# microsoft/Nova

Measured on NVIDIA H100. Metric: MSM throughput (2^20 BN254 scalar*G1/s), higher is better.
Workload: dtype u32 limbs (256-bit prime-field / curve integers)

## Files before the change

### nova_b200/csrc/capi.cu

```cuda
#include <cuda_runtime.h>

#include <algorithm>
#include <atomic>
#include <cstdarg>
#include <cstdio>
#include <cstring>
#include <cstdlib>
#include <map>
#include <memory>
#include <mutex>
#include <vector>

#include "../../include/nova_b200.h"
#include "msm_kernels.cuh"
#include "field_kernels.cuh"
#include "ops.cuh"
#include "poly_kernels.cuh"
#include "transcript.cuh"
#include "transcript_batched.cuh"
#include "sumcheck_tail.cuh"

using namespace nova;

namespace {
// ... 225 lines not shown
size_t acc_lmin() {
  static const size_t lmin = [] {
    const char* e = getenv("NOVA_B200_ACC_LMIN");
    int v = e ? atoi(e) : L_FLOOR_DEFAULT;
    return (size_t)(v < 8 ? 8 : (v > L_MIN ? L_MIN : v));
  }();
  return lmin;
}
int segment_len(size_t entries) {
  size_t L = (entries + acc_threads() - 1) / acc_threads();
  return (int)(L < acc_lmin() ? acc_lmin() : L);
}
size_t max_segments(size_t entries) {
  size_t by_floor = (entries + acc_lmin() - 1) / acc_lmin();
  size_t cap = acc_threads() + 256;
  return by_floor < cap ? by_floor : cap;
}

int ws_acquire(workspace& w, cudaStream_t s) {
  if (w.busy && w.last_stream != s) CU(cudaStreamWaitEvent(s, w.busy, 0));
  return B200_OK;
}
int ws_release(workspace& w, cudaStream_t s) {
  if (!w.busy) CU(cudaEventCreateWithFlags(&w.busy, cudaEventDisableTiming));
  CU(cudaEventRecord(w.busy, s));
  w.last_stream = s;
  return B200_OK;
}

int ensure_workspace(ck_ctx& ck, workspace& w, size_t n, size_t out_slots) {
  if (out_slots > w.out_slots) {
    if (w.d_out) cudaFree(w.d_out);
    if (w.h_out) cudaFreeHost(w.h_out);
    w.d_out = w.h_out = nullptr;
    CU(cudaMalloc(&w.d_out, out_slots * 96));
    CU(cudaMallocHost(&w.h_out, out_slots * 96));
    w.out_slots = out_slots;
  }
  if (n <= w.cap_n) return B200_OK;
  if (n * (size_t)ck.W > 0x7FFFFFFFu)
    return fail(B200_E_RANGE, "%zu scalars x %d windows exceed 2^31 bucket entries", n, ck.W);
  CU(cudaDeviceSynchronize());
  void** szbufs[] = {&w.scalars, (void**)&w.digits, (void**)&w.entries, (void**)&w.entries_tmp, (void**)&w.look,
                     &w.parts, (void**)&w.pkeys, (void**)&w.heavy, &w.hparts};
  for (void** p : szbufs)
    if (*p) {
      cudaFree(*p);
      *p = nullptr;
    }
  size_t K = (size_t)ck.G * ck.B;
  size_t entries = n * (size_t)ck.W;
  size_t nseg = max_segments(entries);
  w.heavy_cap = (uint32_t)(nseg / HEAVY_PARTS + 2);
  CU(cudaMalloc((void**)&w.heavy, ((size_t)w.heavy_cap + 1) * 4));
  CU(cudaMalloc(&w.hparts, (size_t)w.heavy_cap * HEAVY_SPLIT * XYZZ_BYTES));
  CU(cudaMalloc(&w.scalars, n * 32));
  CU(cudaMalloc((void**)&w.digits, entries * sizeof(int32_t)));
  CU(cudaMalloc((void**)&w.entries, entries * sizeof(uint64_t)));
  CU(cudaMalloc((void**)&w.entries_tmp, entries * sizeof(uint64_t)));
  const size_t look_bytes = (entries + SORT_TILE - 1) / SORT_TILE * SORT_BINS * sizeof(unsigned long long);
  CU(cudaMalloc((void**)&w.look, look_bytes));
  CU(cudaMemset(w.look, 0, look_bytes));
  w.sort_epoch = 0;
  CU(cudaMalloc(&w.parts, 2 * nseg * XYZZ_BYTES));
  CU(cudaMalloc((void**)&w.pkeys, 2 * nseg * sizeof(uint32_t)));
  if (!w.sortctl) {
    CU(cudaMalloc((void**)&w.sortctl, SORT_CTL_WORDS * 4));
    CU(cudaMalloc((void**)&w.start, (K + 1) * 4));
    CU(cudaMalloc(&w.buckets, K * XYZZ_BYTES));
    CU(cudaMalloc(&w.rparts, ((size_t)ck.G * (ck.B / ck.m + 4096)) * XYZZ_BYTES));
    CU(cudaMalloc(&w.sumscratch, (size_t)SUM_THREADS * XYZZ_BYTES));
  }
  w.cap_n = n;
  return B200_OK;
}

int ensure_workspace(ck_ctx& ck, size_t n, size_t out_slots) {
  return ensure_workspace(ck, ck.ws, n, out_slots);
}

msm_plan make_plan(ck_ctx& ck, workspace& ws, size_t base_offset, size_t n) {
  msm_plan p;
  p.n = n;
  p.n_ck = ck.stride;
  p.base_offset = base_offset;
  p.blind_i = SIZE_MAX;
  p.h_index = ck.n;
  p.c = ck.c;
  p.W = ck.W;
  p.G = ck.G;
  p.B = ck.B;
  p.L = segment_len(n * (size_t)ck.W);
  p.m = ck.m;
  p.heavy = ws.heavy;
  p.heavy_min = HEAVY_PARTS * (uint32_t)p.L;
  p.heavy_cap = ws.heavy_cap;
  p.hparts = ws.hparts;
  p.digits = ws.digits;
  p.sortctl = ws.sortctl;
  p.sp = make_sort_plan((uint64_t)ck.G * ck.B);
  p.sort_tag = 0;
  p.look = ws.look;
  p.start = ws.start;
  p.entries = ws.entries;
  p.entries_tmp = ws.entries_tmp;
  p.buckets = ws.buckets;
  p.parts = ws.parts;
  p.pkeys = ws.pkeys;
  p.rparts = ws.rparts;
  return p;
}

int enqueue_msm(ck_ctx& ck, workspace& ws, size_t base_offset, const void* d_scalars, size_t n,
                void* d_out, cudaStream_t s, int small_elem_bytes = 0, bool blinded = false,
                bool digits_done = false, const msm_peer* peer = nullptr, bool profile_ok = true) {
  const field_ops* sops = ops_for_field(CURVES[ck.curve].scalar_fid);
  const field_ops* bops = ops_for_field(CURVES[ck.curve].base_fid);
  {
    int arc = ws_acquire(ws, s);
    if (arc) return arc;
  }
  if (n == 0) {
    if (peer && peer->world > 1) {
      msm_plan p0 = make_plan(ck, ws, base_offset, 0);
      p0.peer = *peer;
      bops->exchange_identity(s, p0, d_out);
      count_launch(1);
      CU(cudaGetLastError());
      return B200_OK;
    }
    CU(cudaMemsetAsync(d_out, 0, 96, s));
    return B200_OK;
  }
  msm_plan p = make_plan(ck, ws, base_offset, n);
  if (peer) p.peer = *peer;
  if (blinded) p.blind_i = n - 1;
  if (!digits_done) CU(cudaMemsetAsync(p.sortctl, 0, SORT_CTL_WORDS * 4, s));
  else CU(cudaMemsetAsync(p.sortctl + SORT_PASSES_MAX * SORT_BINS, 0, SORT_PASSES_MAX * 4, s));
  CU(cudaMemsetAsync(p.heavy, 0, 4, s));
  if (ws.sort_epoch > 0x7FFFFFFFu - SORT_PASSES_MAX) {
    CU(cudaMemsetAsync(ws.look, 0, (ws.cap_n * (size_t)ck.W + SORT_TILE - 1) / SORT_TILE * SORT_BINS * 8, s));
    ws.sort_epoch = 0;
  }
  p.sort_tag = ws.sort_epoch + 1;
  ws.sort_epoch += (uint32_t)p.sp.passes;
  std::lock_guard<std::mutex> plk(g_prof.mu);
  const bool prof = g_prof.enabled && profile_ok;
  const int pset = g_prof.next;
  if (prof) {
    if (!g_prof.have_events) {
      for (auto& set : g_prof.ev)
        for (auto& e : set) CU(cudaEventCreate(&e));
      g_prof.have_events = true;
    }
    prof_fold_set_locked(pset);
    g_prof.next = (pset + 1) % profile_state::PROF_RING;
  }
#define STAGE_MARK(i) \
  if (prof) CU(cudaEventRecord(g_prof.ev[pset][i], s))
  STAGE_MARK(ST_DIGITS);
  if (digits_done)
    ;
  else if (small_elem_bytes)
    msm_digits_small(s, d_scalars, small_elem_bytes, p);
  else
    sops->digits(s, d_scalars, p);
  STAGE_MARK(ST_SORT);
  const int sort_launches = msm_sort(s, p);
  STAGE_MARK(ST_ACCUMULATE);
  bops->accumulate(s, ck.tables, p);
  STAGE_MARK(ST_FIXUP);
  bops->fixup(s, p);
  STAGE_MARK(ST_REDUCE);
  bops->reduce(s, p, d_out);
  STAGE_MARK(ST_COUNT);
#undef STAGE_MARK
  if (prof) g_prof.pending[pset] = true;
  for (int i = 0; i < ST_COUNT; i++) g_prof.launches += STAGE_KERNELS[i];
  g_prof.launches += sort_launches - STAGE_KERNELS[ST_SORT];
  g_prof.launches += (ck.c - 1 + 3) / 4 - 1;
  CU(cudaGetLastError());
  return ws_release(ws, s);
}

int enqueue_msm(ck_ctx& ck, size_t base_offset, const void* d_scalars, size_t n, void* d_out,
                cudaStream_t s, int small_elem_bytes = 0, bool blinded = false) {
  return enqueue_msm(ck, ck.ws, base_offset, d_scalars, n, d_out, s, small_elem_bytes, blinded);
}

constexpr size_t SMALL_KEY_MAX = (size_t)1 << 21;
constexpr int SMALL_KEY_WINDOW = 17;

int choose_window(size_t n) {
  int lg = 0;
  while (((size_t)1 << lg) < n) lg++;
  int c = lg;
  if (c < 8) c = 8;
  if (c > 16) c = 16;
  if (lg >= 22) c = 20;
  else if (lg >= 19) c = 17;
  return c;
}

constexpr int CURVE_B_SMALL[4] = {3, -17, 5, 5};

int register_key(int curve_id, const void* bases, bool bases_on_device, size_t n, const void* h,
                 int window_bits, bool expand, std::shared_ptr<ck_ctx>& out, size_t* first_bad = nullptr,
                 cudaStream_t st = nullptr, size_t src_pitch_points = 0, size_t src_block_points = 0) {
  if (!st) st = g_dev.stream;
  if (curve_id < 0 || curve_id > 3) return fail(B200_E_ARG, "unknown curve id %d", curve_id);
  if (bases == nullptr || n == 0) return fail(B200_E_ARG, "empty commitment key");
  if (window_bits != 0 && (window_bits < 2 || window_bits > 24))
    return fail(B200_E_ARG, "window_bits %d out of range [2,24]", window_bits);
  auto ck = std::make_shared<ck_ctx>();
  ck->curve = curve_id;
  ck->n = n;
  ck->has_h = h != nullptr;
  ck->stride = n + (h ? 1 : 0);
  ck->c = window_bits ? window_bits : choose_window(n);
  int bits = FIELD_BITS[CURVES[curve_id].scalar_fid];
  ck->W = (bits + ck->c - 1) / ck->c;
  ck->F = expand ? ck->W : 1;
  ck->G = expand ? 1 : ck->W;
  ck->B = 1u << (ck->c - 1);
  ck->m = ck->B >= 4 ? 4 : 1;
  if ((size_t)ck->F * ck->stride >= ((size_t)1 << 31))
    return fail(B200_E_RANGE, "key too large for 31-bit table indices (%zu x %d)", n, ck->F);
  CU(cudaMalloc(&ck->tables, (size_t)ck->F * ck->stride * 64));
  const cudaMemcpyKind kind = bases_on_device ? cudaMemcpyDeviceToDevice : cudaMemcpyHostToDevice;
  if (src_block_points == 0) {
    CU(cudaMemcpyAsync(ck->tables, bases, n * 64, kind, st));
  } else {
    const size_t full = n / src_block_points, rest = n % src_block_points;
// ... 1400 lines not shown
```

### nova_b200/csrc/curve.cuh

```cuda
#pragma once
#include "field.cuh"

namespace nova {

struct xyzz_t {
  fe_t x, y, zz, zzz;
};

struct affine_t {
  fe_t x, y;
};

template <class F>
NOVA_HD xyzz_t xyzz_identity() {
  xyzz_t r;
  r.x = fe_one<F>();
  r.y = fe_one<F>();
  r.zz = fe_zero<F>();
  r.zzz = fe_zero<F>();
  return r;
}

NOVA_HD bool xyzz_is_identity(const xyzz_t& p) { return fe_is_zero(p.zz); }
NOVA_HD bool affine_is_identity(const affine_t& p) { return fe_is_zero(p.x) && fe_is_zero(p.y); }
// ... 90 lines not shown
    if (fe_eq(s1, s2))
      xyzz_dbl<F>(acc);
    else
      acc = xyzz_identity<F>();
    return;
  }
  fe_t p = fe_sub<F>(u2, u1);
  fe_t r = fe_sub<F>(s2, s1);
  fe_t pp = fe_sqr<F>(p);
  fe_t ppp = fe_mul<F>(p, pp);
  fe_t q = fe_mul<F>(u1, pp);
  fe_t x3 = fe_sub<F>(fe_sub<F>(fe_sqr<F>(r), ppp), fe_dbl<F>(q));
  fe_t y3 = fe_sub<F>(fe_mul<F>(r, fe_sub<F>(q, x3)), fe_mul<F>(s1, ppp));
  acc.x = x3;
  acc.y = y3;
  acc.zz = fe_mul<F>(fe_mul<F>(acc.zz, o.zz), pp);
  acc.zzz = fe_mul<F>(fe_mul<F>(acc.zzz, o.zzz), ppp);
}

template <class F>
NOVA_HD void xyzz_neg(xyzz_t& p) {
  p.y = fe_neg<F>(p.y);
}

template <class F>
NOVA_HD void xyzz_to_jacobian(const xyzz_t& p, fe_t& X, fe_t& Y, fe_t& Z) {
  if (xyzz_is_identity(p)) {
    X = fe_zero<F>();
    Y = fe_one<F>();
    Z = fe_zero<F>();
    return;
  }
  fe_t zzz2 = fe_sqr<F>(p.zzz);
  fe_t zz_zzz2 = fe_mul<F>(p.zz, zzz2);
  X = fe_mul<F>(p.x, zz_zzz2);
  fe_t zz2 = fe_sqr<F>(p.zz);
  Y = fe_mul<F>(p.y, fe_mul<F>(zz2, zz_zzz2));
  Z = fe_mul<F>(p.zz, p.zzz);
}

template <class F>
NOVA_HD xyzz_t xyzz_mul_small(const xyzz_t& p, uint32_t k) {
  xyzz_t acc = xyzz_identity<F>();
  if (k == 0 || xyzz_is_identity(p)) return acc;
  int top = 31;
  while (!((k >> top) & 1)) top--;
  for (int i = top; i >= 0; i--) {
    xyzz_dbl<F>(acc);
    if ((k >> i) & 1) xyzz_add<F>(acc, p);
  }
  return acc;
}

#if defined(__CUDACC__)
NOVA_D affine_t affine_load(const void* base, size_t idx) {
  affine_t a;
  a.x = fe_load(base, 2 * idx);
  a.y = fe_load(base, 2 * idx + 1);
  return a;
}
NOVA_D xyzz_t xyzz_load(const void* base, size_t idx) {
  xyzz_t p;
  p.x = fe_load_rw(base, 4 * idx);
  p.y = fe_load_rw(base, 4 * idx + 1);
  p.zz = fe_load_rw(base, 4 * idx + 2);
  p.zzz = fe_load_rw(base, 4 * idx + 3);
  return p;
}
NOVA_D void xyzz_store(void* base, size_t idx, const xyzz_t& p) {
  fe_store(base, 4 * idx, p.x);
  fe_store(base, 4 * idx + 1, p.y);
  fe_store(base, 4 * idx + 2, p.zz);
  fe_store(base, 4 * idx + 3, p.zzz);
}
#endif

}
```

### nova_b200/csrc/msm_kernels.cuh

```cuda
#pragma once
#include <cuda_runtime.h>
#include "curve29.cuh"
#include "coop.cuh"
#include "msm_sort.cuh"

namespace nova {

constexpr uint32_t KEY_INVALID = 0xffffffffu;

constexpr int MSM_PEER_MAX = 8;
constexpr size_t MSM_PEER_FLAGS_OFF = (size_t)2 * MSM_PEER_MAX * 128;
constexpr size_t MSM_PEER_ERR_OFF = MSM_PEER_FLAGS_OFF + (size_t)MSM_PEER_MAX * 8;
constexpr size_t MSM_PEER_BUF_BYTES = MSM_PEER_ERR_OFF + 8;
struct msm_peer {
  int world = 1, rank = 0;
  unsigned long long epoch = 0;
  void* buf[MSM_PEER_MAX] = {};
};

struct msm_plan {
  size_t n;
  size_t n_ck;
  size_t base_offset;
  size_t blind_i;
  size_t h_index;
  int c;
  int W;
  int G;
  uint32_t B;
  int L;
  int m;
  int32_t* digits;
  uint32_t* sortctl;
  sort_plan sp;
  uint32_t sort_tag;
  unsigned long long* look;
  uint32_t* start;
  uint64_t* entries;
  uint64_t* entries_tmp;
  void* buckets;
  void* parts;
  uint32_t* pkeys;
  void* rparts;
  uint32_t* heavy;
  uint32_t heavy_min;
  uint32_t heavy_cap;
  void* hparts;
  msm_peer peer;
};

template <class S>
__global__ void __launch_bounds__(256) k_digits(const void* __restrict__ scalars, size_t i0, size_t i1,
                                                size_t n, int c, int W, int G, uint32_t B,
                                                int32_t* __restrict__ digits,
                                                uint32_t* __restrict__ hist, const sort_plan sp) {
  __shared__ uint32_t s_hist[SORT_PASSES_MAX * SORT_BINS];
  sort_hist_clear(s_hist);
  for (size_t blk = i0 + (size_t)blockIdx.x * blockDim.x; blk < i1; blk += (size_t)gridDim.x * blockDim.x) {
    size_t i = blk + threadIdx.x;
    const bool live = i < i1;
    fe_t s = live ? fe_from_mont<S>(fe_load(scalars, i)) : fe_zero<S>();
    uint32_t p[8], t[8];
    load_p<S>(p);
    bool neg = false;
    if (!fe_is_zero(s)) {
      sub8(t, p, s.l);
      uint32_t d[8];
      uint32_t lt = sub8(d, t, s.l);
      if (lt) {
        neg = true;
#pragma unroll
        for (int k = 0; k < 8; k++) s.l[k] = t[k];
      }
    }
    const uint32_t half = 1u << (c - 1);
    const uint32_t mask = (1u << c) - 1;
    uint32_t carry = 0;
    for (int w = 0; w < W; w++) {
      int bit = w * c;
      int limb = bit >> 5, sh = bit & 31;
      uint32_t v = 0;
      if (limb < 8) {
        uint64_t two = s.l[limb];
        if (limb + 1 < 8) two |= (uint64_t)s.l[limb + 1] << 32;
        v = (uint32_t)(two >> sh) & mask;
      }
      v += carry;
      int32_t dgt;
      if (v > half) {
        dgt = (int32_t)v - (int32_t)(1u << c);
        carry = 1;
      } else {
        dgt = (int32_t)v;
        carry = 0;
      }
      if (neg) dgt = -dgt;
      if (live) digits[(size_t)w * n + i] = dgt;
      uint32_t key = NO_KEY;
      if (dgt != 0) {
        uint32_t mag = dgt < 0 ? (uint32_t)(-dgt) : (uint32_t)dgt;
        key = (uint32_t)(w % G) * B + (mag - 1);
      }
// ... 643 lines not shown
  for (int s = 32; s > 0; s >>= 1) {
    if (quad < s && s < nsplit) {
      xyzz_t o = sm[quad + s];
      coop_add<F>(acc, o, cm);
    }
    __syncthreads();
    if (quad < s && cm.lane() == 0) sm[quad] = acc;
    __syncthreads();
  }
  if (threadIdx.x == 0) xyzz_store(merged, ((size_t)g * lv.nd + d) * 16 + v, acc);
}

template <class F>
NOVA_D xyzz_t peer_exchange_sum(const xyzz_t& mine, const msm_peer& peer, xyzz_t* sm ,
                                const quad_comm_dev& cm) {
  const int tid = threadIdx.x, quad = tid >> 2;
  const int set = (int)(peer.epoch & 1ull);
  if (tid == 0) sm[0] = mine;
  __syncthreads();
  if (tid < peer.world) {
    char* dst = (char*)peer.buf[tid];
    xyzz_store(dst, (size_t)set * MSM_PEER_MAX + peer.rank, sm[0]);
    __threadfence_system();
    volatile unsigned long long* flag = (volatile unsigned long long*)(dst + MSM_PEER_FLAGS_OFF) + peer.rank;
    *flag = peer.epoch;
    char* loc = (char*)peer.buf[peer.rank];
    const unsigned long long* lflag = (const unsigned long long*)(loc + MSM_PEER_FLAGS_OFF) + tid;
    unsigned long long seen = 0;
    long long t0 = clock64();
    for (;;) {
      asm volatile("ld.acquire.sys.global.u64 %0, [%1];" : "=l"(seen) : "l"(lflag) : "memory");
      if (seen >= peer.epoch) break;
      if (clock64() - t0 > (1ll << 32)) {
        *(volatile unsigned long long*)(loc + MSM_PEER_ERR_OFF) = peer.epoch;
        break;
      }
    }
  }
  __syncthreads();
  xyzz_t acc = xyzz_identity<F>();
  if (quad < peer.world) acc = xyzz_load((const char*)peer.buf[peer.rank], (size_t)set * MSM_PEER_MAX + quad);
  for (int s = MSM_PEER_MAX / 2; s > 0; s >>= 1) {
    if (quad < 2 * s && cm.lane() == 0) sm[quad] = acc;
    __syncthreads();
    if (quad < s && quad + s < peer.world) {
      xyzz_t o = sm[quad + s];
      coop_add<F>(acc, o, cm);
    }
    __syncthreads();
  }
  return acc;
}

template <class F>
__global__ void __launch_bounds__(384) k_red_final_q(const void* __restrict__ merged, int G, int bits, int c,
                                                     void* __restrict__ out_jac, const msm_peer peer) {
  __shared__ xyzz_t sm[96];
  quad_comm_dev cm;
  const int nd = (bits + 3) / 4;
  const int quad = threadIdx.x >> 2;
  const int d = quad >> 4, v = quad & 15;
  xyzz_t total = xyzz_identity<F>();
  for (int g = G - 1; g >= 0; g--) {
    xyzz_t acc = xyzz_identity<F>();
    if (d < nd) acc = xyzz_load(merged, ((size_t)g * nd + d) * 16 + v);
    if (cm.lane() == 0) sm[quad] = acc;
    __syncthreads();
    for (int dd = 1; dd < 16; dd <<= 1) {
      bool have = v + dd < 16;
      xyzz_t o = xyzz_identity<F>();
      if (have) o = sm[quad + dd];
      __syncthreads();
      if (have) coop_add<F>(acc, o, cm);
      if (cm.lane() == 0) sm[quad] = acc;
      __syncthreads();
    }
    xyzz_t t0 = acc;
    if (v == 0) acc = xyzz_identity<F>();
    if (cm.lane() == 0) sm[quad] = acc;
    __syncthreads();
    for (int s = 8; s > 0; s >>= 1) {
      bool have = v < s;
      xyzz_t o = xyzz_identity<F>();
      if (have) o = sm[quad + s];
      __syncthreads();
      if (have) coop_add<F>(acc, o, cm);
      if (cm.lane() == 0) sm[quad] = acc;
      __syncthreads();
    }
    if (v == 0 && d < nd) {
      for (int i = 0; i < 4 * d; i++) coop_dbl<F>(acc, cm);
      if (d == 0) coop_add<F>(acc, t0, cm);
      if (cm.lane() == 0) sm[quad] = acc;
    }
    __syncthreads();
    if (quad == 0) {
      if (g != G - 1)
        for (int i = 0; i < c; i++) coop_dbl<F>(total, cm);
      for (int dd = 0; dd < nd; dd++) {
        xyzz_t o = sm[dd * 16];
        coop_add<F>(total, o, cm);
      }
    }
    __syncthreads();
  }
  if (peer.world > 1) total = peer_exchange_sum<F>(total, peer, sm, cm);
  if (threadIdx.x == 0) {
    fe_t X, Y, Z;
    xyzz_to_jacobian<F>(total, X, Y, Z);
    fe_store(out_jac, 0, X);
    fe_store(out_jac, 1, Y);
    fe_store(out_jac, 2, Z);
  }
}
#endif

template <class F>
__global__ void k_jacobian_sum(const void* __restrict__ pts, int k, void* __restrict__ out_jac) {
  using PA = msm_arith<F>;
  if (blockIdx.x != 0 || threadIdx.x != 0) return;
  typename PA::pt acc = PA::identity();
  for (int i = 0; i < k; i++) {
    fe_t X = fe_load(pts, 3 * (size_t)i), Y = fe_load(pts, 3 * (size_t)i + 1),
         Z = fe_load(pts, 3 * (size_t)i + 2);
    typename PA::pt p = PA::from_jacobian_std(X, Y, Z);
    PA::add(acc, p);
  }
  fe_t X, Y, Z;
  PA::to_jacobian_std(acc, X, Y, Z);
  fe_store(out_jac, 0, X);
  fe_store(out_jac, 1, Y);
  fe_store(out_jac, 2, Z);
}

#if !defined(NOVA_MSM_ARITH29)
template <class F>
__global__ void __launch_bounds__(32) k_jacobian_sum_q(const void* __restrict__ pts, int k, void* __restrict__ out_jac) {
  __shared__ xyzz_t sm[8];
  quad_comm_dev cm;
  const int quad = threadIdx.x >> 2;
  xyzz_t acc = xyzz_identity<F>();
  for (int i = quad; i < k; i += 8) {
    fe_t X = fe_load(pts, 3 * (size_t)i), Y = fe_load(pts, 3 * (size_t)i + 1), Z = fe_load(pts, 3 * (size_t)i + 2);
    xyzz_t p = xyzz_identity<F>();
    if (!fe_is_zero(Z)) {
      p.x = X;
      p.y = Y;
      p.zz = fe_sqr<F>(Z);
      p.zzz = fe_mul<F>(p.zz, Z);
    }
    coop_add<F>(acc, p, cm);
  }
  for (int s = 4; s > 0; s >>= 1) {
    if (quad < 2 * s && cm.lane() == 0) sm[quad] = acc;
    __syncwarp();
    if (quad < s) {
      xyzz_t o = sm[quad + s];
      coop_add<F>(acc, o, cm);
// ... 127 lines not shown
```

### nova_b200/csrc/ops.cuh

```cuda
#pragma once
#include <cstdlib>
#include <cuda_runtime.h>
#include <cstddef>
#include <cstdint>

namespace nova {

struct msm_plan;
struct multi_args;
struct poly_multi_args;
struct scb_tail_args;
struct spark_mats;
struct r1cs_mats;

struct field_ops {
  int field_id;
  void (*digits)(cudaStream_t, const void* scalars, const msm_plan&);
  void (*expand_key)(cudaStream_t, void* tables, size_t n_ck, int ntables, int shift);
  void (*accumulate)(cudaStream_t, const void* tables, const msm_plan&);
  void (*fixup)(cudaStream_t, const msm_plan&);
  void (*reduce)(cudaStream_t, const msm_plan&, void* out_jac);
  void (*sum_points)(cudaStream_t, const void* tables, const uint32_t* idx_or_null, size_t n,
                     void* scratch_xyzz, void* out_jac);
  void (*jacobian_sum)(cudaStream_t, const void* pts, int k, void* out_jac);
  void (*index_bases)(cudaStream_t, void* bases, size_t n, const void* gen_affine, uint64_t k0);
  void (*cross_term)(cudaStream_t, const void* az, const void* bz, const void* cz, const void* e1,
                     const void* e2_or_null, const void* u, size_t n, void* t);
  void (*axpy)(cudaStream_t, const void* a, const void* b, const void* r, size_t n, void* out);
  void (*vec_add)(cudaStream_t, const void* a, const void* b, size_t n, void* out);
  void (*bind_top)(cudaStream_t, void* z, size_t n, const void* r);
  void (*bind_top_multi)(cudaStream_t, void* const* zs, int k, size_t n, const void* r);
  void (*vec_mul)(cudaStream_t, const void* a, const void* b, size_t n, void* out);
  void (*logup_hash)(cudaStream_t, const void* val, const void* addr_or_null, const void* gamma,
                     const void* r, size_t n, void* out);
  void (*fold_halves)(cudaStream_t, const void* v, size_t half, const void* x_lo, const void* x_hi, void* out);
  void (*ipa_scalars)(cudaStream_t, const void* a, const void* w, size_t n, size_t nk, void* sL, void* sR);
  void (*ipa_weights)(cudaStream_t, void* w, size_t n, size_t nk, const void* r, const void* r_inv);
  void (*fill_one)(cudaStream_t, void* w, size_t n);
  void (*sc_reduce)(cudaStream_t, int form, const void* A, const void* B, const void* C, size_t count,
                    size_t half, const void* eq_left, const void* eq_right, int shift, size_t id_mul,
                    size_t id_add, void* scratch, void* out);
  void (*eq_small)(cudaStream_t, const void* r, int ell, void* out);
  void (*eq_outer)(cudaStream_t, const void* left, const void* right, int right_bits, size_t n,
                   void* out);
  void (*batch_invert)(cudaStream_t, const void* in, size_t n, void* out, int* zero_flag);
  void (*rlc)(cudaStream_t, const void* const* polys, const size_t* lens, int k, const void* coeffs,
              size_t n, void* out);
  void (*kzg_fold)(cudaStream_t, const void* p, const void* x, size_t half, void* out);
  void (*poly_eval)(cudaStream_t, const void* f, size_t n, const void* us, int nu, void* scratch,
                    void* evals);
  void (*poly_div)(cudaStream_t, const void* f, size_t n, size_t cols, const void* u, void* scratch, void* out,
                   void* rem_or_null);
  void (*spmv_classify)(cudaStream_t, const void* vals, size_t nnz, int8_t* codes);
  void (*spmv)(cudaStream_t, const uint32_t* indptr, const uint32_t* cols, const int8_t* codes,
               const void* vals, size_t rows, const void* z1, const void* z2_or_null, void* o1,
               void* o2_or_null);
  void (*spmv_t)(cudaStream_t, const uint32_t* tptr, const uint32_t* trow, const uint32_t* tperm,
                 const int8_t* codes, const void* vals, size_t cols, size_t out_len, const void* rx,
                 void* out);
  void (*sc_round)(cudaStream_t, int kind, void* state, const void* res, const void* tau,
                   const void* tau_inv, const void* pending, uint32_t pending_len, int absorb_label,
                   int squeeze_label, void* out_poly, void* out_r);
  void (*fe_inv_each)(cudaStream_t, const void* in, size_t n, void* out);
  void (*digits_range)(cudaStream_t, const void* scalars, size_t i0, size_t i1, const msm_plan&);
  void (*sc_round_batched)(cudaStream_t, const void* desc, void* state, const void* sums, const void* pending,
                           uint32_t pending_len, int absorb_label, int squeeze_label, void* out_poly, void* out_r);
  void (*on_curve)(cudaStream_t, const void* pts, size_t n, int b_small, uint32_t* first_bad);
  void (*powers_canonical)(cudaStream_t, const void* u_mont, size_t n, void* out);
  void (*scalar_bases)(cudaStream_t, void* bases, size_t n, const void* gen_affine, const void* scalars_canonical);
  void (*poseidon_ro)(cudaStream_t, int t, int r_f, int r_p, const void* rc, const void* mds, const void* elems, uint32_t n,
                      const void* tag_canonical, int num_bits, int start_with_one, void* out);
  void (*to_mont)(cudaStream_t, const void* in_canonical, size_t n, void* out);
  void (*exchange_identity)(cudaStream_t, const msm_plan&, void* out_jac);
  void (*sc_round_batched_fused)(cudaStream_t, const void* desc, void* state, const void* partials, int nblocks,
// ... 78 lines not shown
```

### nova_b200/csrc/ops_impl.cuh

```cuda
#pragma once
#include "ops.cuh"
#include "msm_kernels.cuh"
#include "field_kernels.cuh"
#include "poly_kernels.cuh"
#include "transcript.cuh"
#include "transcript_batched.cuh"
#include "poseidon.cuh"
#include "sumcheck_tail.cuh"

namespace nova {

inline int stream_grid(size_t n, int block, int waves = 8) {
  size_t need = (n + block - 1) / block;
  size_t cap = (size_t)NUM_SMS * waves;
  size_t g = need < cap ? need : cap;
  return (int)(g == 0 ? 1 : g);
}

template <class F>
__global__ void __launch_bounds__(128) k_sum_points1(const void* __restrict__ tables,
                                                     const uint32_t* __restrict__ idx, size_t n,
                                                     void* __restrict__ partial) {
  size_t tid = (size_t)blockIdx.x * blockDim.x + threadIdx.x;
  size_t nthreads = (size_t)gridDim.x * blockDim.x;
// ... 22 lines not shown
    int block = 128;
    int grid = (int)((n_ck + block - 1) / block);
    k_expand_key<F><<<grid, block, 0, s>>>(tables, n_ck, ntables, shift);
  }
  static void accumulate(cudaStream_t s, const void* tables, const msm_plan& p) {
    uint32_t K = (uint32_t)p.G * p.B;
    size_t max_entries = p.n * (size_t)p.W;
    size_t nseg = (max_entries + p.L - 1) / p.L;
    int block = 128;
    int grid = (int)((nseg + block - 1) / block);
#if !defined(NOVA_MSM_ARITH29)
    static const bool use_tma = [] {
      const char* e = getenv("NOVA_B200_ACC_TMA");
      return e != nullptr && e[0] == '1';
    }();
    if (use_tma) {
      k_accumulate_tma<F><<<grid, block, 0, s>>>(p.entries, p.start, K, tables, p.L, p.buckets, p.parts, p.pkeys);
      return;
    }
#endif
    k_accumulate<F><<<grid, block, 0, s>>>(p.entries, p.start, K, tables, p.L, p.buckets, p.parts,
                                           p.pkeys);
  }
  static void fixup(cudaStream_t s, const msm_plan& p) {
    uint32_t K = (uint32_t)p.G * p.B;
    size_t entries = p.n * (size_t)p.W;
    size_t ppk = entries / ((size_t)K * p.L) + 1;
    int G = 1;
    while (G < 32 && (size_t)G * 8 < ppk) G <<= 1;
    if (ppk <= 16) G = 1;
    size_t threads = (size_t)K * G;
#if !defined(NOVA_MSM_ARITH29)
    if (G == 1) {
      threads = (size_t)K * 4;
      k_fixup_q<F><<<(unsigned)((threads + 127) / 128), 128, 0, s>>>(p.start, K, p.L, p.heavy_min, p.parts,
                                                                     p.pkeys, p.buckets);
    } else
#endif
      k_fixup<F><<<(unsigned)((threads + 127) / 128), 128, 0, s>>>(p.start, K, p.L, p.heavy_min, G, p.parts,
                                                                   p.pkeys, p.buckets);
    k_fixup_heavy1<F><<<NUM_SMS * 4, 256, 0, s>>>(p.start, p.L, p.heavy, p.parts, p.pkeys, p.hparts);
    k_fixup_heavy2<F><<<NUM_SMS, 32, 0, s>>>(p.heavy, p.hparts, p.buckets);
  }
  static void index_bases(cudaStream_t s, void* bases, size_t n, const void* gen, uint64_t k0) {
    k_index_bases<F><<<(unsigned)((n + 127) / 128), 128, 0, s>>>(bases, n, gen, k0);
  }
  static void jacobian_sum(cudaStream_t s, const void* pts, int k, void* out_jac) {
#if !defined(NOVA_MSM_ARITH29)
    k_jacobian_sum_q<F><<<1, 32, 0, s>>>(pts, k, out_jac);
#else
    k_jacobian_sum<F><<<1, 32, 0, s>>>(pts, k, out_jac);
#endif
  }
  static void reduce(cudaStream_t s, const msm_plan& p, void* out_jac) {
    int bits = p.c - 1;
#if !defined(NOVA_MSM_ARITH29)
    static const int flat_mode = [] {
      const char* e = getenv("NOVA_B200_RED_FLAT");
      return e == nullptr ? -1 : (e[0] == '1' ? 1 : 0);
    }();
    static const int hier_bits = [] {
      const char* e = getenv("NOVA_B200_RED_HIER_BITS");
      return e ? atoi(e) : 18;
    }();
    const bool flat = flat_mode == 1 || (flat_mode == -1 && bits < hier_bits);
    if (bits >= 1 && bits <= 24 && !flat) {
      red_levels lv{};
      lv.nd = (bits + 3) / 4;
      size_t off = 0;
      uint32_t N = p.B;
      const void* X = p.buckets;
      for (int l = 0; l < lv.nd - 1; l++) {
        const uint32_t groups = N >> 4;
        int nsplit = (int)((groups + 511) / 512);
        if (nsplit < 1) nsplit = 1;
        lv.nsplit[l] = nsplit;
        lv.parts_off[l] = (unsigned)off;
        char* parts = (char*)p.rparts + off * 128;
        off += (size_t)p.G * 16 * nsplit;
        char* next = (char*)p.rparts + off * 128;
        const unsigned next_off = (unsigned)off;
        off += (size_t)p.G * groups;
        unsigned gx = (unsigned)nsplit, gb = (groups + 15) / 16;
        dim3 grid(gx > gb ? gx : gb, 17u, (unsigned)p.G);
        k_red_level_q<F><<<grid, 256, 0, s>>>(l == 0 ? p.start : nullptr, p.B, X, N, nsplit, parts, next);
        X = next;
        N = groups;
        lv.top_off = next_off;
      }
      if (lv.nd == 1) lv.top_off = 0xFFFFFFFFu;
      lv.top_n = N;
      char* merged = (char*)p.rparts + off * 128;
      dim3 g2((unsigned)(lv.nd * 16), (unsigned)p.G);
      k_red_merge_levels_q<F><<<g2, 256, 0, s>>>(p.rparts, lv, p.start, p.B, p.buckets, p.G, merged);
      k_red_final_q<F><<<1, 384, 0, s>>>(merged, p.G, bits, p.c, out_jac, p.peer);
      return;
    }
    if (bits >= 1 && bits <= 24) {
      int nd = (bits + 3) / 4;
      uint32_t count = p.B >> (bits < 4 ? bits : 4);
      int nsplit = (int)((count + 255) / 256);
      if (nsplit < 1) nsplit = 1;
      if (nsplit > 4096) nsplit = 4096;
      char* merged = (char*)p.rparts + (size_t)p.G * nd * 16 * nsplit * 128;
      dim3 g1((unsigned)nsplit, (unsigned)(nd * 16), (unsigned)p.G);
      k_red_digits_q<F><<<g1, 256, 0, s>>>(p.start, p.B, bits, p.buckets, p.rparts);
      dim3 g2((unsigned)(nd * 16), (unsigned)p.G);
      k_red_merge_q<F><<<g2, 256, 0, s>>>(p.rparts, nd, nsplit, merged);
      k_red_final_q<F><<<1, 384, 0, s>>>(merged, p.G, bits, p.c, out_jac, p.peer);
      return;
    }
#endif
    if (bits >= 1 && bits <= 24) {
      int nd = (bits + 3) / 4;
      dim3 g1(RED_NSPLIT, (unsigned)(nd * 16), (unsigned)p.G);
      k_red_digits<F><<<g1, 128, 0, s>>>(p.start, p.B, bits, p.buckets, p.rparts);
      k_red_final<F><<<1, 256, 0, s>>>(p.rparts, p.G, bits, p.c, out_jac);
      return;
    }
    uint32_t T = p.B / p.m;
    int block = 128;
    int grid = (int)(((size_t)T * p.G + block - 1) / block);
    k_reduce1<F><<<grid, block, 0, s>>>(p.start, p.B, p.G, p.m, p.buckets, p.rparts);
    k_reduce2<F><<<1, 256, 0, s>>>(p.rparts, T, p.G, p.c, out_jac);
  }
  static void sum_points(cudaStream_t s, const void* tables, const uint32_t* idx, size_t n,
                         void* scratch, void* out_jac) {
    int block = 128, grid = NUM_SMS;
    k_sum_points1<F><<<grid, block, 0, s>>>(tables, idx, n, scratch);
    k_reduce2<F><<<1, 256, 0, s>>>(scratch, (uint32_t)(grid * block), 1, 0, out_jac);
  }
  static void cross_term(cudaStream_t s, const void* az, const void* bz, const void* cz,
                         const void* e1, const void* e2, const void* u, size_t n, void* t) {
    k_cross_term<F><<<stream_grid(n, 256), 256, 0, s>>>(az, bz, cz, e1, e2, u, n, t);
  }
  static void axpy(cudaStream_t s, const void* a, const void* b, const void* r, size_t n,
                   void* out) {
    k_axpy<F><<<stream_grid(n, 256), 256, 0, s>>>(a, b, r, n, out);
  }
  static void vec_add(cudaStream_t s, const void* a, const void* b, size_t n, void* out) {
    k_vec_add<F><<<stream_grid(n, 256), 256, 0, s>>>(a, b, n, out);
  }
  static void vec_mul(cudaStream_t s, const void* a, const void* b, size_t n, void* out) {
    k_vec_mul<F><<<stream_grid(n, 256), 256, 0, s>>>(a, b, n, out);
  }
  static void logup_hash(cudaStream_t s, const void* val, const void* addr, const void* gamma,
                         const void* r, size_t n, void* out) {
    k_logup_hash<F><<<stream_grid(n, 256), 256, 0, s>>>(val, addr, gamma, r, n, out);
  }
  static void bind_top(cudaStream_t s, void* z, size_t n, const void* r) {
    k_bind_top<F><<<stream_grid(n / 2, 256), 256, 0, s>>>(z, n / 2, r);
  }
  static void bind_top_multi(cudaStream_t s, void* const* zs, int k, size_t n, const void* r) {
    bind_multi_args a{};
    for (int i = 0; i < k; i++) a.z[i] = zs[i];
    int gx = stream_grid(n / 2, 256, 8);
    int per = (NUM_SMS * 8 + k - 1) / k;
    if (gx > per) gx = per < 1 ? 1 : per;
    k_bind_top_multi<F><<<dim3((unsigned)gx, (unsigned)k), 256, 0, s>>>(a, n / 2, r);
  }
  static void fold_halves(cudaStream_t s, const void* v, size_t half, const void* x_lo, const void* x_hi,
                          void* out) {
    k_fold_halves<F><<<stream_grid(half, 256), 256, 0, s>>>(v, half, x_lo, x_hi, out);
  }
  static void ipa_scalars(cudaStream_t s, const void* a, const void* w, size_t n, size_t nk, void* sL,
                          void* sR) {
    k_ipa_scalars<F><<<stream_grid(n, 256), 256, 0, s>>>(a, w, n, nk, sL, sR);
  }
  static void ipa_weights(cudaStream_t s, void* w, size_t n, size_t nk, const void* r, const void* r_inv) {
    k_ipa_weights<F><<<stream_grid(n, 256), 256, 0, s>>>(w, n, nk, r, r_inv);
  }
  static void fill_one(cudaStream_t s, void* w, size_t n) {
    k_fill_one<F><<<stream_grid(n, 256), 256, 0, s>>>(w, n);
  }
  template <int FORM>
  static void sc_launch(cudaStream_t s, const void* A, const void* B, const void* C, size_t count,
                        size_t half, const void* eq_left, const void* eq_right, int shift,
// ... 228 lines not shown
    if (n) k_on_curve<F><<<stream_grid(n, 256), 256, 0, s>>>(pts, n, b_small, first_bad);
  }
  static void powers_canonical(cudaStream_t s, const void* u, size_t n, void* out) {
    if (n) k_powers_canonical<F><<<(unsigned)((n + 127) / 128), 128, 0, s>>>(u, n, out);
  }
  static void scalar_bases(cudaStream_t s, void* bases, size_t n, const void* gen, const void* scalars) {
    if (n) k_scalar_bases<F><<<(unsigned)((n + 127) / 128), 128, 0, s>>>(bases, n, gen, scalars);
  }
  static void poseidon_ro(cudaStream_t s, int t, int r_f, int r_p, const void* rc, const void* mds, const void* elems,
                          uint32_t n, const void* tag, int num_bits, int start_with_one, void* out) {
    poseidon_desc d{t, r_f, r_p};
    k_poseidon_ro<F><<<1, 32 * t, 0, s>>>(d, rc, mds, elems, n, tag, num_bits, start_with_one, out);
  }
  static void to_mont(cudaStream_t s, const void* in, size_t n, void* out) {
    if (n) k_to_mont<F><<<(unsigned)((n + 255) / 256), 256, 0, s>>>(in, n, out);
  }
  static void exchange_identity(cudaStream_t s, const msm_plan& p, void* out_jac) {
#if !defined(NOVA_MSM_ARITH29)
    k_red_final_q<F><<<1, 384, 0, s>>>(nullptr, 0, 4, 4, out_jac, p.peer);
#endif
  }
  static void derive_check(cudaStream_t s, const void* tables, size_t n, const uint32_t* addr, size_t m,
                           size_t table_size, uint32_t* flags) {
    if (n) k_derive_check<F><<<stream_grid(n, 256), 256, 0, s>>>(tables, n, addr, m, table_size, flags);
  }
  static void derive_affine(cudaStream_t s, const uint32_t* start, uint32_t K, const void* buckets, void* out) {
    if (K) k_derive_affine<F><<<(unsigned)((K + 127) / 128), 128, 0, s>>>(start, K, buckets, out);
  }
  static void r1cs_eval(cudaStream_t s, const r1cs_mats& m, int k, const void* tx, const void* ty, void* scratch,
                        void* out) {
    size_t nnz = 0;
    for (int y = 0; y < k; y++) nnz = m.nnz[y] > nnz ? m.nnz[y] : nnz;
    const size_t want = (nnz + 256 * R1CS_MIN_CHUNK - 1) / (256 * R1CS_MIN_CHUNK);
    const unsigned gx = (unsigned)(want < 1 ? 1 : (want > R1CS_EVAL_BLOCKS ? R1CS_EVAL_BLOCKS : want));
    const size_t threads = (size_t)gx * 256, chunk = nnz ? (nnz + threads - 1) / threads : 1;
    k_r1cs_eval<F><<<dim3(gx, (unsigned)k), 256, 0, s>>>(m, tx, ty, chunk, scratch);
    k_r1cs_final<F><<<dim3(1, (unsigned)k), 256, 0, s>>>(scratch, (int)gx, out);
  }
  static void ipa_s(cudaStream_t s, const void* r, const void* r_inv, int L, const void* scale, void* scratch,
                    void* out) {
    if (L <= IPA_S_DIRECT_BITS) {
      k_ipa_s_half<F><<<(unsigned)((((size_t)1 << L) + 255) / 256), 256, 0, s>>>(r, r_inv, L, scale, out);
      return;
    }
    const int rb = L / 2, lb = L - rb;
    void* left = scratch;
    void* right = (char*)scratch + ((size_t)32 << lb);
    k_ipa_s_half<F><<<(unsigned)((((size_t)1 << lb) + 255) / 256), 256, 0, s>>>(r, r_inv, lb, scale, left);
    k_ipa_s_half<F><<<(unsigned)((((size_t)1 << rb) + 255) / 256), 256, 0, s>>>(
        (const char*)r + 32 * lb, (const char*)r_inv + 32 * lb, rb, nullptr, right);
    k_eq_outer<F><<<stream_grid((size_t)1 << L, 256), 256, 0, s>>>(left, right, rb, (size_t)1 << L, out);
  }
  static constexpr field_ops table() {
    return field_ops{F::ID,  digits,       expand_key, accumulate, fixup,   reduce,
                     sum_points, jacobian_sum, index_bases, cross_term, axpy,       vec_add, bind_top, bind_top_multi, vec_mul, logup_hash,
                     fold_halves, ipa_scalars, ipa_weights, fill_one,
                     sc_reduce, eq_small, eq_outer, batch_invert, rlc, kzg_fold, poly_eval, poly_div, spmv_classify, spmv, spmv_t,
                     sc_round, fe_inv_each, digits_range, sc_round_batched, on_curve,
                     powers_canonical, scalar_bases, poseidon_ro, to_mont, exchange_identity,
                     sc_round_batched_fused, sc_reduce_multi_partials, gather_heads, poly_eval_small_multi,
                     eq_prefix_tables, sc_reduce_multi, scb_tail, mat_vec_rows, mercury_s_poly,
                     neutron_evals, pow_split_evals, lerp, spark_repr, derive_check, derive_affine, r1cs_eval, ipa_s};
  }
};

}
```

Baseline: 286.1 million.

## Fuse MSM bucket fixup and reduction into a two-kernel tail

Replaces the separate fixup pass and the multi-kernel bucket reduction with a two-kernel tail for window widths 13-16 on a single device. The first kernel joins segment partial sums into buckets and reduces spans of buckets into per-digit partials, also handling heavy-bucket splits. The second kernel merges the per-digit partials and uses an atomic ticket so the last block runs the final group combination, removing the single-block launch. This cuts kernel launches and the intermediate writes of bucket fixup, at the cost of a linear scan over segment keys per bucket and a last-block serialization.

```diff
diff --git a/nova_b200/csrc/capi.cu b/nova_b200/csrc/capi.cu
--- a/nova_b200/csrc/capi.cu
+++ b/nova_b200/csrc/capi.cu
@@ -301,7 +301,8 @@
   size_t entries = n * (size_t)ck.W;
   size_t nseg = max_segments(entries);
   w.heavy_cap = (uint32_t)(nseg / HEAVY_PARTS + 2);
-  CU(cudaMalloc((void**)&w.heavy, ((size_t)w.heavy_cap + 1) * 4));
+  CU(cudaMalloc((void**)&w.heavy, ((size_t)w.heavy_cap + 2) * 4));
+  CU(cudaMemset(w.heavy, 0, ((size_t)w.heavy_cap + 2) * 4));
   CU(cudaMalloc(&w.hparts, (size_t)w.heavy_cap * HEAVY_SPLIT * XYZZ_BYTES));
   CU(cudaMalloc(&w.scalars, n * 32));
   CU(cudaMalloc((void**)&w.digits, entries * sizeof(int32_t)));
@@ -345,6 +346,7 @@
   p.heavy_min = HEAVY_PARTS * (uint32_t)p.L;
   p.heavy_cap = ws.heavy_cap;
   p.hparts = ws.hparts;
+  p.ticket = ws.heavy + ws.heavy_cap + 1;
   p.digits = ws.digits;
   p.sortctl = ws.sortctl;
   p.sp = make_sort_plan((uint64_t)ck.G * ck.B);
@@ -419,15 +421,15 @@
   STAGE_MARK(ST_ACCUMULATE);
   bops->accumulate(s, ck.tables, p);
   STAGE_MARK(ST_FIXUP);
-  bops->fixup(s, p);
+  const bool fused = msm_tail_fused(p.c - 1) && p.peer.world == 1;
+  if (!fused) bops->fixup(s, p);
   STAGE_MARK(ST_REDUCE);
-  bops->reduce(s, p, d_out);
+  const int reduce_launches = fused ? bops->tail(s, p, d_out) : bops->reduce(s, p, d_out);
   STAGE_MARK(ST_COUNT);
 #undef STAGE_MARK
   if (prof) g_prof.pending[pset] = true;
-  for (int i = 0; i < ST_COUNT; i++) g_prof.launches += STAGE_KERNELS[i];
-  g_prof.launches += sort_launches - STAGE_KERNELS[ST_SORT];
-  g_prof.launches += (ck.c - 1 + 3) / 4 - 1;
+  g_prof.launches += STAGE_KERNELS[ST_DIGITS] + sort_launches + STAGE_KERNELS[ST_ACCUMULATE] +
+                     (fused ? 0 : STAGE_KERNELS[ST_FIXUP]) + reduce_launches;
   CU(cudaGetLastError());
   return ws_release(ws, s);
 }
diff --git a/nova_b200/csrc/curve.cuh b/nova_b200/csrc/curve.cuh
--- a/nova_b200/csrc/curve.cuh
+++ b/nova_b200/csrc/curve.cuh
@@ -166,7 +166,7 @@
   return acc;
 }
 
-#if defined(__CUDACC__)
+#if defined(__CUDACC__) || defined(NOVA_SIMT_HOST)
 NOVA_D affine_t affine_load(const void* base, size_t idx) {
   affine_t a;
   a.x = fe_load(base, 2 * idx);
diff --git a/nova_b200/csrc/msm_kernels.cuh b/nova_b200/csrc/msm_kernels.cuh
--- a/nova_b200/csrc/msm_kernels.cuh
+++ b/nova_b200/csrc/msm_kernels.cuh
@@ -46,8 +46,21 @@
   uint32_t heavy_min;
   uint32_t heavy_cap;
   void* hparts;
+  uint32_t* ticket;
   msm_peer peer;
 };
+
+inline bool msm_tail_fused(int bits) {
+#if defined(NOVA_MSM_ARITH29)
+  return false;
+#else
+  static const bool split = [] {
+    const char* e = getenv("NOVA_B200_TAIL_SPLIT");
+    return e != nullptr && e[0] == '1';
+  }();
+  return !split && bits >= 13 && bits <= 16;
+#endif
+}
 
 template <class S>
 __global__ void __launch_bounds__(256) k_digits(const void* __restrict__ scalars, size_t i0, size_t i1,
@@ -797,58 +810,16 @@
   return acc;
 }
 
+}
+#include "msm_tail.cuh"
+namespace nova {
+
 template <class F>
 __global__ void __launch_bounds__(384) k_red_final_q(const void* __restrict__ merged, int G, int bits, int c,
                                                      void* __restrict__ out_jac, const msm_peer peer) {
   __shared__ xyzz_t sm[96];
   quad_comm_dev cm;
-  const int nd = (bits + 3) / 4;
-  const int quad = threadIdx.x >> 2;
-  const int d = quad >> 4, v = quad & 15;
-  xyzz_t total = xyzz_identity<F>();
-  for (int g = G - 1; g >= 0; g--) {
-    xyzz_t acc = xyzz_identity<F>();
-    if (d < nd) acc = xyzz_load(merged, ((size_t)g * nd + d) * 16 + v);
-    if (cm.lane() == 0) sm[quad] = acc;
-    __syncthreads();
-    for (int dd = 1; dd < 16; dd <<= 1) {
-      bool have = v + dd < 16;
-      xyzz_t o = xyzz_identity<F>();
-      if (have) o = sm[quad + dd];
-      __syncthreads();
-      if (have) coop_add<F>(acc, o, cm);
-      if (cm.lane() == 0) sm[quad] = acc;
-      __syncthreads();
-    }
-    xyzz_t t0 = acc;
-    if (v == 0) acc = xyzz_identity<F>();
-    if (cm.lane() == 0) sm[quad] = acc;
-    __syncthreads();
-    for (int s = 8; s > 0; s >>= 1) {
-      bool have = v < s;
-      xyzz_t o = xyzz_identity<F>();
-      if (have) o = sm[quad + s];
-      __syncthreads();
-      if (have) coop_add<F>(acc, o, cm);
-      if (cm.lane() == 0) sm[quad] = acc;
-      __syncthreads();
-    }
-    if (v == 0 && d < nd) {
-      for (int i = 0; i < 4 * d; i++) coop_dbl<F>(acc, cm);
-      if (d == 0) coop_add<F>(acc, t0, cm);
-      if (cm.lane() == 0) sm[quad] = acc;
-    }
-    __syncthreads();
-    if (quad == 0) {
-      if (g != G - 1)
-        for (int i = 0; i < c; i++) coop_dbl<F>(total, cm);
-      for (int dd = 0; dd < nd; dd++) {
-        xyzz_t o = sm[dd * 16];
-        coop_add<F>(total, o, cm);
-      }
-    }
-    __syncthreads();
-  }
+  xyzz_t total = red_final_groups<F>(merged, G, bits, c, sm, cm);
   if (peer.world > 1) total = peer_exchange_sum<F>(total, peer, sm, cm);
   if (threadIdx.x == 0) {
     fe_t X, Y, Z;
diff --git a/nova_b200/csrc/msm_tail.cuh b/nova_b200/csrc/msm_tail.cuh
--- /dev/null
+++ b/nova_b200/csrc/msm_tail.cuh
@@ -0,0 +1,209 @@
+#pragma once
+
+namespace nova {
+
+constexpr int TAIL_SPAN_BITS = 8;
+
+template <class F, class Comm>
+NOVA_D xyzz_t quad_block_sum(xyzz_t acc, uint32_t n, xyzz_t* sm, const Comm& cm) {
+  const int quad = threadIdx.x >> 2;
+  if (cm.lane() == 0) sm[quad] = acc;
+  __syncthreads();
+  for (int s = 32; s > 0; s >>= 1) {
+    if (quad < s && (uint32_t)s < n) {
+      xyzz_t o = sm[quad + s];
+      coop_add<F>(acc, o, cm);
+    }
+    __syncthreads();
+    if (quad < s && cm.lane() == 0) sm[quad] = acc;
+    __syncthreads();
+  }
+  return acc;
+}
+
+template <class F, class Comm>
+NOVA_D xyzz_t red_final_groups(const void* merged, int G, int bits, int c, xyzz_t* sm, const Comm& cm) {
+  const int nd = (bits + 3) / 4;
+  const int quad = threadIdx.x >> 2;
+  const int d = quad >> 4, v = quad & 15;
+  xyzz_t total = xyzz_identity<F>();
+  for (int g = G - 1; g >= 0; g--) {
+    xyzz_t acc = xyzz_identity<F>();
+    if (d < nd) acc = xyzz_load(merged, ((size_t)g * nd + d) * 16 + v);
+    if (cm.lane() == 0) sm[quad] = acc;
+    __syncthreads();
+    for (int dd = 1; dd < 16; dd <<= 1) {
+      bool have = v + dd < 16;
+      xyzz_t o = xyzz_identity<F>();
+      if (have) o = sm[quad + dd];
+      __syncthreads();
+      if (have) coop_add<F>(acc, o, cm);
+      if (cm.lane() == 0) sm[quad] = acc;
+      __syncthreads();
+    }
+    xyzz_t t0 = acc;
+    if (v == 0) acc = xyzz_identity<F>();
+    if (cm.lane() == 0) sm[quad] = acc;
+    __syncthreads();
+    for (int s = 8; s > 0; s >>= 1) {
+      bool have = v < s;
+      xyzz_t o = xyzz_identity<F>();
+      if (have) o = sm[quad + s];
+      __syncthreads();
+      if (have) coop_add<F>(acc, o, cm);
+      if (cm.lane() == 0) sm[quad] = acc;
+      __syncthreads();
+    }
+    if (v == 0 && d < nd) {
+      for (int i = 0; i < 4 * d; i++) coop_dbl<F>(acc, cm);
+      if (d == 0) coop_add<F>(acc, t0, cm);
+      if (cm.lane() == 0) sm[quad] = acc;
+    }
+    __syncthreads();
+    if (quad == 0) {
+      if (g != G - 1)
+        for (int i = 0; i < c; i++) coop_dbl<F>(total, cm);
+      for (int dd = 0; dd < nd; dd++) {
+        xyzz_t o = sm[dd * 16];
+        coop_add<F>(total, o, cm);
+      }
+    }
+    __syncthreads();
+  }
+  return total;
+}
+
+template <class F>
+__global__ void __launch_bounds__(256) k_tail_join_q(const uint32_t* __restrict__ start, int bits, int L,
+                                                     uint32_t heavy_min, const void* __restrict__ parts,
+                                                     const uint32_t* __restrict__ pkeys,
+                                                     const void* __restrict__ buckets,
+                                                     const uint32_t* __restrict__ heavy, void* __restrict__ hparts,
+                                                     void* __restrict__ bparts) {
+  __shared__ xyzz_t sm[256];
+  quad_comm_dev cm;
+  const int quad = threadIdx.x >> 2;
+  const int span = bits < TAIL_SPAN_BITS ? bits : TAIL_SPAN_BITS;
+  const uint32_t key0 = (uint32_t)blockIdx.x << span;
+  for (int i = quad; i < 256; i += 64) {
+    xyzz_t acc = xyzz_identity<F>();
+    if (i < (1 << span)) {
+      const uint32_t key = key0 + (uint32_t)i;
+      const uint32_t s0 = start[key], s1 = start[key + 1];
+      if (s1 != s0 && s1 - s0 <= heavy_min) {
+        const size_t j0 = 2 * ((size_t)s0 / L), j1 = 2 * (((size_t)s1 - 1) / L) + 1;
+        bool found = false;
+        for (size_t j = j0; j <= j1; j++) {
+          if (pkeys[j] == key) {
+            xyzz_t o = xyzz_load(parts, j);
+            coop_add<F>(acc, o, cm);
+            found = true;
+          }
+        }
+        if (!found) acc = xyzz_load(buckets, key);
+      }
+    }
+    if (cm.lane() == 0) sm[i] = acc;
+  }
+  __syncthreads();
+  {
+    const int o = quad >> 1, h = quad & 1;
+    xyzz_t acc = xyzz_identity<F>();
+    for (int m = 0; m < 8; m++) {
+      const int t = 8 * h + m;
+      xyzz_t x = sm[o < 16 ? 16 * t + o : 16 * (o - 16) + t];
+      coop_add<F>(acc, x, cm);
+    }
+    __syncthreads();
+    if (h == 1 && cm.lane() == 0) sm[o] = acc;
+    __syncthreads();
+    if (h == 0) {
+      xyzz_t x = sm[o];
+      coop_add<F>(acc, x, cm);
+      if (cm.lane() == 0) xyzz_store(bparts, (size_t)blockIdx.x * 32 + o, acc);
+    }
+  }
+  const uint32_t nitems = heavy[0] * HEAVY_SPLIT;
+  for (uint32_t it = blockIdx.x; it < nitems; it += gridDim.x) {
+    __syncthreads();
+    const uint32_t key = heavy[1 + it / HEAVY_SPLIT], sl = it % HEAVY_SPLIT;
+    const size_t s0 = 2 * ((size_t)start[key] / L);
+    const size_t s1 = 2 * (((size_t)start[key + 1] - 1) / L) + 2;
+    const size_t per = (s1 - s0 + HEAVY_SPLIT - 1) / HEAVY_SPLIT;
+    const size_t lo = s0 + sl * per, hi = lo + per < s1 ? lo + per : s1;
+    xyzz_t acc = xyzz_identity<F>();
+    for (size_t j = lo + quad; j < hi; j += 64) {
+      if (pkeys[j] == key) {
+        xyzz_t o = xyzz_load(parts, j);
+        coop_add<F>(acc, o, cm);
+      }
+    }
+    acc = quad_block_sum<F>(acc, 64, sm, cm);
+    if (threadIdx.x == 0) xyzz_store(hparts, it, acc);
+  }
+}
+
+template <class F>
+__global__ void __launch_bounds__(256) k_tail_final_q(const void* __restrict__ bparts,
+                                                      const uint32_t* __restrict__ heavy,
+                                                      const void* __restrict__ hparts, uint32_t B, int bits, int c,
+                                                      int G, void* __restrict__ merged, uint32_t* __restrict__ ticket,
+                                                      void* __restrict__ out_jac, const msm_peer peer) {
+  __shared__ xyzz_t sm[64];
+  __shared__ bool last;
+  quad_comm_dev cm;
+  const int quad = threadIdx.x >> 2;
+  const int nd = (bits + 3) / 4;
+  const int span = bits < TAIL_SPAN_BITS ? bits : TAIL_SPAN_BITS;
+  const uint32_t nblk = B >> span;
+  const uint32_t g = blockIdx.x / (nd * 16);
+  const int d = (int)(blockIdx.x % (nd * 16)) >> 4, v = (int)(blockIdx.x & 15);
+  const int width = bits - 4 * d < 4 ? bits - 4 * d : 4;
+  const uint32_t n_in = v < (1 << width) ? (d < 2 ? nblk : (nblk >> width) * 16) : 0;
+  const int sh = 4 * (d - 2);
+  const uint32_t nh = heavy[0] * HEAVY_SPLIT;
+  xyzz_t acc = xyzz_identity<F>();
+  for (uint32_t t = quad; t < n_in + nh; t += 64) {
+    size_t idx;
+    if (t < n_in) {
+      if (d < 2) {
+        idx = ((size_t)g * nblk + t) * 32 + 16 * d + v;
+      } else {
+        const uint32_t u = t >> 4;
+        const uint32_t k = ((u >> sh) << (sh + width)) | ((uint32_t)v << sh) | (u & ((1u << sh) - 1));
+        idx = ((size_t)g * nblk + k) * 32 + (t & 15);
+      }
+      xyzz_t o = xyzz_load(bparts, idx);
+      coop_add<F>(acc, o, cm);
+    } else {
+      const uint32_t it = t - n_in, key = heavy[1 + it / HEAVY_SPLIT];
+      if (key / B == g && (((key % B) >> (4 * d)) & 15) == (uint32_t)v) {
+        xyzz_t o = xyzz_load(hparts, it);
+        coop_add<F>(acc, o, cm);
+      }
+    }
+  }
+  acc = quad_block_sum<F>(acc, n_in + nh, sm, cm);
+  if (threadIdx.x == 0) {
+    xyzz_store(merged, ((size_t)g * nd + d) * 16 + v, acc);
+    __threadfence();
+    last = atomicAdd(ticket, 1u) == gridDim.x - 1;
+  }
+  __syncthreads();
+  if (!last) return;
+  __threadfence();
+  if (threadIdx.x == 0) *ticket = 0;
+  xyzz_t total = red_final_groups<F>(merged, G, bits, c, sm, cm);
+#if !defined(NOVA_SIMT_HOST)
+  if (peer.world > 1) total = peer_exchange_sum<F>(total, peer, sm, cm);
+#endif
+  if (threadIdx.x == 0) {
+    fe_t X, Y, Z;
+    xyzz_to_jacobian<F>(total, X, Y, Z);
+    fe_store(out_jac, 0, X);
+    fe_store(out_jac, 1, Y);
+    fe_store(out_jac, 2, Z);
+  }
+}
+
+}
diff --git a/nova_b200/csrc/ops.cuh b/nova_b200/csrc/ops.cuh
--- a/nova_b200/csrc/ops.cuh
+++ b/nova_b200/csrc/ops.cuh
@@ -19,7 +19,8 @@
   void (*expand_key)(cudaStream_t, void* tables, size_t n_ck, int ntables, int shift);
   void (*accumulate)(cudaStream_t, const void* tables, const msm_plan&);
   void (*fixup)(cudaStream_t, const msm_plan&);
-  void (*reduce)(cudaStream_t, const msm_plan&, void* out_jac);
+  int (*reduce)(cudaStream_t, const msm_plan&, void* out_jac);
+  int (*tail)(cudaStream_t, const msm_plan&, void* out_jac);
   void (*sum_points)(cudaStream_t, const void* tables, const uint32_t* idx_or_null, size_t n,
                      void* scratch_xyzz, void* out_jac);
   void (*jacobian_sum)(cudaStream_t, const void* pts, int k, void* out_jac);
diff --git a/nova_b200/csrc/ops_impl.cuh b/nova_b200/csrc/ops_impl.cuh
--- a/nova_b200/csrc/ops_impl.cuh
+++ b/nova_b200/csrc/ops_impl.cuh
@@ -98,7 +98,23 @@
     k_jacobian_sum<F><<<1, 32, 0, s>>>(pts, k, out_jac);
 #endif
   }
-  static void reduce(cudaStream_t s, const msm_plan& p, void* out_jac) {
+  static int tail(cudaStream_t s, const msm_plan& p, void* out_jac) {
+#if !defined(NOVA_MSM_ARITH29)
+    const int bits = p.c - 1, nd = (bits + 3) / 4;
+    const int span = bits < TAIL_SPAN_BITS ? bits : TAIL_SPAN_BITS;
+    const unsigned nblk = (unsigned)(((size_t)p.G * p.B) >> span);
+    char* merged = (char*)p.rparts + (size_t)nblk * 32 * 128;
+    k_tail_join_q<F><<<nblk, 256, 0, s>>>(p.start, bits, p.L, p.heavy_min, p.parts, p.pkeys, p.buckets, p.heavy,
+                                          p.hparts, p.rparts);
+    k_tail_final_q<F><<<(unsigned)(p.G * nd * 16), 256, 0, s>>>(p.rparts, p.heavy, p.hparts, p.B, bits, p.c, p.G,
+                                                                merged, p.ticket, out_jac, p.peer);
+    return 2;
+#else
+    (void)s, (void)p, (void)out_jac;
+    return 0;
+#endif
+  }
+  static int reduce(cudaStream_t s, const msm_plan& p, void* out_jac) {
     int bits = p.c - 1;
 #if !defined(NOVA_MSM_ARITH29)
     static const int flat_mode = [] {
@@ -140,7 +156,7 @@
       dim3 g2((unsigned)(lv.nd * 16), (unsigned)p.G);
       k_red_merge_levels_q<F><<<g2, 256, 0, s>>>(p.rparts, lv, p.start, p.B, p.buckets, p.G, merged);
       k_red_final_q<F><<<1, 384, 0, s>>>(merged, p.G, bits, p.c, out_jac, p.peer);
-      return;
+      return lv.nd + 1;
     }
     if (bits >= 1 && bits <= 24) {
       int nd = (bits + 3) / 4;
@@ -154,7 +170,7 @@
       dim3 g2((unsigned)(nd * 16), (unsigned)p.G);
       k_red_merge_q<F><<<g2, 256, 0, s>>>(p.rparts, nd, nsplit, merged);
       k_red_final_q<F><<<1, 384, 0, s>>>(merged, p.G, bits, p.c, out_jac, p.peer);
-      return;
+      return 3;
     }
 #endif
     if (bits >= 1 && bits <= 24) {
@@ -162,13 +178,14 @@
       dim3 g1(RED_NSPLIT, (unsigned)(nd * 16), (unsigned)p.G);
       k_red_digits<F><<<g1, 128, 0, s>>>(p.start, p.B, bits, p.buckets, p.rparts);
       k_red_final<F><<<1, 256, 0, s>>>(p.rparts, p.G, bits, p.c, out_jac);
-      return;
+      return 2;
     }
     uint32_t T = p.B / p.m;
     int block = 128;
     int grid = (int)(((size_t)T * p.G + block - 1) / block);
     k_reduce1<F><<<grid, block, 0, s>>>(p.start, p.B, p.G, p.m, p.buckets, p.rparts);
     k_reduce2<F><<<1, 256, 0, s>>>(p.rparts, T, p.G, p.c, out_jac);
+    return 2;
   }
   static void sum_points(cudaStream_t s, const void* tables, const uint32_t* idx, size_t n,
                          void* scratch, void* out_jac) {
@@ -503,7 +520,7 @@
     k_eq_outer<F><<<stream_grid((size_t)1 << L, 256), 256, 0, s>>>(left, right, rb, (size_t)1 << L, out);
   }
   static constexpr field_ops table() {
-    return field_ops{F::ID,  digits,       expand_key, accumulate, fixup,   reduce,
+    return field_ops{F::ID,  digits,       expand_key, accumulate, fixup,   reduce, tail,
                      sum_points, jacobian_sum, index_bases, cross_term, axpy,       vec_add, bind_top, bind_top_multi, vec_mul, logup_hash,
                      fold_halves, ipa_scalars, ipa_weights, fill_one,
                      sc_reduce, eq_small, eq_outer, batch_invert, rlc, kzg_fold, poly_eval, poly_div, spmv_classify, spmv, spmv_t,
```

Measured after the change: 291.4 million, median of 6. 1.9% higher.
